# eriklindernoren/PyTorch-GAN

Measured on NVIDIA H100. Metric: DCGAN 64x64 images/sec (full G+D step), higher is better.
Workload: dtype tf32 (fp32 storage, fp32 accumulate)

## Files before the change

### include/b200gan.h

```cpp
#ifndef B200GAN_H
#define B200GAN_H

#include <stddef.h>
#include <stdint.h>

#ifdef __cplusplus
extern "C" {
#endif

#define B200GAN_VERSION 100

enum {
  B200GAN_OK = 0,
  B200GAN_E_UNSUPPORTED = -1,
  B200GAN_E_BAD_ARG = -2,
  B200GAN_E_CUDA = -3,
  B200GAN_E_ARCH = -4
};

enum { B200GAN_ACT_NONE = 0, B200GAN_ACT_LRELU = 1, B200GAN_ACT_RELU = 2, B200GAN_ACT_TANH = 3,
       B200GAN_ACT_SIGMOID = 4 };

enum { B200GAN_ALGO_AUTO = 0,
       B200GAN_ALGO_SIMT = 1,
// ... 32 lines not shown
  int32_t round_tf32;
} b200gan_epilogue;

int b200gan_version(void);
const char *b200gan_last_error(void);
int b200gan_check_device(void);

size_t b200gan_packed_weight_floats(const b200gan_conv_geom *g, int pack);
int b200gan_pack_weights(const b200gan_conv_geom *g, int pack, const float *w, float *packed,
                         void *stream);

typedef struct b200gan_pack_job {
  const float *w;
  float *packed;
  b200gan_conv_geom geom;
  int32_t pack;
} b200gan_pack_job;
int b200gan_pack_weights_multi(const b200gan_pack_job *jobs, int32_t count, void *stream);

int b200gan_conv2d_supported(const b200gan_conv_geom *g, int pass, int algo);

int b200gan_conv2d_fprop(const b200gan_conv_geom *g, const b200gan_epilogue *ep, const float *x,
                         const float *packed, float *y, int algo, void *stream);

size_t b200gan_conv2d_dgrad_workspace_floats(const b200gan_conv_geom *g, int algo);
int b200gan_conv2d_dgrad(const b200gan_conv_geom *g, const float *dy, const float *packed,
                         float *dx, float *workspace, int algo, void *stream);

size_t b200gan_conv2d_wgrad_workspace_floats(const b200gan_conv_geom *g, int algo);
int b200gan_conv2d_wgrad(const b200gan_conv_geom *g, const float *x, const float *dy, float *dw,
                         float *db, float *workspace, int algo, void *stream);
int b200gan_conv2d_wgrad_fused_bias(const b200gan_conv_geom *g, const float *x, const float *dy, float *dw,
                                    float *db, float *workspace, int algo, void *stream);

int b200gan_epilogue_bwd(const float *dy, const float *y, const float *chan_scale, int32_t act,
                         float slope, int64_t n, int32_t K, int64_t PQ, int32_t round_tf32,
                         float *dz, void *stream);

int b200gan_bias_grad(const float *dy, const float *y, const float *chan_scale, int32_t act, float slope,
                      int64_t rows, int32_t K, int64_t PQ, float *db, void *stream);

typedef struct b200gan_norm_desc {
  int32_t N, HW, C;
  int32_t per_sample;
  float eps;
  float momentum;
  int32_t act;
  float slope;
  int32_t round_tf32;
} b200gan_norm_desc;

int b200gan_norm_stats(const b200gan_norm_desc *d, const float *x, double *stats, void *stream);
int b200gan_norm_finalize(const b200gan_norm_desc *d, double *stats, const float *gamma,
                          const float *beta, float *mean_rstd, float *scale_shift,
                          float *running_mean, float *running_var, int64_t *num_batches_tracked,
                          void *stream);
int b200gan_norm_apply(const b200gan_norm_desc *d, const float *x, const float *scale_shift,
                       float *y, void *stream);
int b200gan_norm_bwd(const b200gan_norm_desc *d, const float *dy, const float *x, const float *y,
                     const float *mean_rstd, const float *scale_shift, const float *gamma, double *sums, float *dx,
                     float *dgamma_dbeta, void *stream);

int b200gan_norm_dbwd(const b200gan_norm_desc *d, const float *dy, const float *x, const float *mean_rstd,
                      const float *scale_shift, const float *gamma, const float *u, const float *ugamma_ubeta,
                      double *sums, float *gx, float *gdy, float *ggamma_per_group, void *stream);

// ... 172 lines not shown
```

### pytorch-gan_b200/b200gan/_lib.py

```python
import ctypes
import os

_HERE = os.path.dirname(os.path.abspath(__file__))
LIB_PATH = os.path.join(_HERE, "libb200gan.so")

c_i32, c_i64, c_f32, c_f64 = ctypes.c_int32, ctypes.c_int64, ctypes.c_float, ctypes.c_double
c_vp, c_sz = ctypes.c_void_p, ctypes.c_size_t

ACT_NONE, ACT_LRELU, ACT_RELU, ACT_TANH, ACT_SIGMOID = 0, 1, 2, 3, 4
ALGO_AUTO, ALGO_SIMT, ALGO_TC = 0, 1, 2
PAD_ZERO, PAD_REFLECT = 0, 1
PACK_SIMT_FPROP, PACK_SIMT_DGRAD, PACK_TC_FPROP, PACK_TC_DGRAD, PACK_TC_FPROP_UP2, PACK_TC_DGRAD_UP2 = range(6)


class ConvGeom(ctypes.Structure):
    _fields_ = [(n, c_i32) for n in (
        "N", "H", "W", "C", "K", "R", "S", "stride", "pad_t", "pad_l", "pad_b", "pad_r",
        "pad_mode", "up", "transposed", "P", "Q")]

    def key(self):
        return tuple(getattr(self, n) for n, _ in self._fields_)


class Epilogue(ctypes.Structure):
# ... 38 lines not shown
class TailDesc(ctypes.Structure):
    _fields_ = [("N", c_i32), ("H", c_i32), ("W", c_i32), ("C", c_i32), ("K", c_i32), ("act_mid", c_i32),
                ("slope", c_f32), ("act_out", c_i32)]


PIXEL_LOSS_MSE, PIXEL_LOSS_L1 = 0, 1
LAYOUT_NCHW, LAYOUT_NHWC = 0, 1


class PixelLossDesc(ctypes.Structure):
    _fields_ = [("mode", c_i32), ("layout_a", c_i32), ("layout_b", c_i32), ("reserved", c_i32), ("n", c_i64),
                ("N", c_i32), ("C", c_i32), ("H", c_i32), ("W", c_i32)]


class AdamTensor(ctypes.Structure):
    _fields_ = [("p", c_vp), ("g", c_vp), ("m", c_vp), ("v", c_vp), ("n", c_i64)]


_P = ctypes.POINTER
SIGNATURES = {
    "b200gan_version": (c_i32, []),
    "b200gan_last_error": (ctypes.c_char_p, []),
    "b200gan_check_device": (c_i32, []),
    "b200gan_packed_weight_floats": (c_sz, [_P(ConvGeom), c_i32]),
    "b200gan_pack_weights": (c_i32, [_P(ConvGeom), c_i32, c_vp, c_vp, c_vp]),
    "b200gan_pack_weights_multi": (c_i32, [_P(PackJob), c_i32, c_vp]),
    "b200gan_conv2d_supported": (c_i32, [_P(ConvGeom), c_i32, c_i32]),
    "b200gan_conv2d_fprop": (c_i32, [_P(ConvGeom), _P(Epilogue), c_vp, c_vp, c_vp, c_i32, c_vp]),
    "b200gan_conv2d_dgrad_workspace_floats": (c_sz, [_P(ConvGeom), c_i32]),
    "b200gan_conv2d_dgrad": (c_i32, [_P(ConvGeom), c_vp, c_vp, c_vp, c_vp, c_i32, c_vp]),
    "b200gan_conv2d_wgrad_workspace_floats": (c_sz, [_P(ConvGeom), c_i32]),
    "b200gan_conv2d_wgrad": (c_i32, [_P(ConvGeom), c_vp, c_vp, c_vp, c_vp, c_vp, c_i32, c_vp]),
    "b200gan_conv2d_wgrad_fused_bias": (c_i32, [_P(ConvGeom), c_vp, c_vp, c_vp, c_vp, c_vp, c_i32, c_vp]),
    "b200gan_epilogue_bwd": (c_i32, [c_vp, c_vp, c_vp, c_i32, c_f32, c_i64, c_i32, c_i64, c_i32, c_vp, c_vp]),
    "b200gan_bias_grad": (c_i32, [c_vp, c_vp, c_vp, c_i32, c_f32, c_i64, c_i32, c_i64, c_vp, c_vp]),
    "b200gan_norm_stats": (c_i32, [_P(NormDesc), c_vp, c_vp, c_vp]),
    "b200gan_norm_finalize": (c_i32, [_P(NormDesc), c_vp, c_vp, c_vp, c_vp, c_vp, c_vp, c_vp, c_vp, c_vp]),
    "b200gan_norm_apply": (c_i32, [_P(NormDesc), c_vp, c_vp, c_vp, c_vp]),
    "b200gan_norm_bwd": (c_i32, [_P(NormDesc), c_vp, c_vp, c_vp, c_vp, c_vp, c_vp, c_vp, c_vp, c_vp, c_vp]),
    "b200gan_norm_dbwd": (c_i32, [_P(NormDesc)] + [c_vp] * 12),
    "b200gan_conv2d_dgrad_norm_supported": (c_i32, [_P(ConvGeom)]),
    "b200gan_conv2d_dgrad_norm": (c_i32, [_P(ConvGeom), _P(NormDesc)] + [c_vp] * 8),
    "b200gan_norm_bwd_from_sums": (c_i32, [_P(NormDesc)] + [c_vp] * 9),
    "b200gan_tail_supported": (c_i32, [_P(TailDesc)]),
    "b200gan_tail_fprop": (c_i32, [_P(TailDesc), c_vp, c_vp, c_vp, c_vp, c_vp, c_vp]),
    "b200gan_tail_bwd_workspace_bytes": (c_sz, [_P(TailDesc)]),
    "b200gan_tail_bwd": (c_i32, [_P(TailDesc)] + [c_vp] * 10 + [c_i32, c_vp]),
    "b200gan_nchw_to_nhwc": (c_i32, [c_vp, c_vp, c_i32, c_i32, c_i32, c_vp]),
    "b200gan_nhwc_to_nchw": (c_i32, [c_vp, c_vp, c_i32, c_i32, c_i32, c_vp]),
    "b200gan_upsample2x_fwd": (c_i32, [c_vp, c_vp, c_i32, c_i32, c_i32, c_i32, c_vp]),
    "b200gan_upsample2x_bwd": (c_i32, [c_vp, c_vp, c_i32, c_i32, c_i32, c_i32, c_vp]),
    "b200gan_pad2d_fwd": (c_i32, [c_vp, c_vp] + [c_i32] * 10 + [c_vp]),
    "b200gan_pad2d_bwd": (c_i32, [c_vp, c_vp] + [c_i32] * 9 + [c_vp]),
    "b200gan_act_fwd": (c_i32, [c_vp, c_vp, c_i32, c_i32, c_f32, c_i64, c_i32, c_i64, c_vp, c_vp]),
    "b200gan_mlp_critic_fwd": (c_i32, [_P(MlpCriticDesc)] + [c_vp] * 13),
    "b200gan_mlp_critic_bwd_workspace_floats": (c_sz, [_P(MlpCriticDesc)]),
    "b200gan_mlp_critic_bwd": (c_i32, [_P(MlpCriticDesc)] + [c_vp] * 20),
    "b200gan_mlp_critic_dbwd_workspace_floats": (c_sz, [_P(MlpCriticDesc)]),
    "b200gan_mlp_critic_dbwd": (c_i32, [_P(MlpCriticDesc)] + [c_vp] * 15),
    "b200gan_critic_step_workspace_floats": (c_sz, [_P(MlpCriticDesc)]),
    "b200gan_critic_step_mlp": (c_i32, [_P(MlpCriticDesc), c_f32] + [c_vp] * 18),
    "b200gan_mlp_disc_fwd": (c_i32, [_P(MlpCriticDesc)] + [c_vp] * 13),
    "b200gan_mlp_disc_bwd_workspace_floats": (c_sz, [_P(MlpCriticDesc)]),
    "b200gan_mlp_disc_bwd": (c_i32, [_P(MlpCriticDesc)] + [c_vp] * 19),
    "b200gan_mlp_gen_saved_floats": (c_sz, [_P(MlpGenDesc)]),
    "b200gan_mlp_gen_workspace_floats": (c_sz, [_P(MlpGenDesc)]),
# ... 56 lines not shown
```

### pytorch-gan_b200/b200gan/ops.py

```python
import ctypes
import os

import torch

from . import _lib
from ._lib import (ACT_NONE, ALGO_AUTO, ALGO_SIMT, ALGO_TC, PACK_SIMT_DGRAD, PACK_SIMT_FPROP, PACK_TC_DGRAD,
                   PACK_TC_DGRAD_UP2, PACK_TC_FPROP, PACK_TC_FPROP_UP2, PAD_REFLECT, PAD_ZERO, ConvGeom, Epilogue,
                   MlpCriticDesc, MlpGenDesc, MlpGenGrads, NbBn, NormDesc, PixelLossDesc, TailDesc)

CL = torch.channels_last


class Config:
    algo = os.environ.get("B200GAN_ALGO", "auto")
    weight_cache = True
    contiguous_hw_limit = 64
    fuse_narrow_chain = os.environ.get("B200GAN_FUSE_CHAIN", "1") not in ("", "0")


def _stream():
    return torch.cuda.current_stream().cuda_stream


def _ptr(t):
# ... 106 lines not shown
def conv_fprop(g, x, packed, algo, bias=None, act=ACT_NONE, slope=0.0, chan_scale=None, stats=None,
               stats_per_sample=False, round_tf32=False):
    y = empty_cl(g.N, g.K, g.P, g.Q, x.device)
    if g.N == 0:
        return y
    ep = Epilogue()
    ep.bias, ep.act, ep.slope = _ptr(bias), act, slope
    ep.chan_scale, ep.stats = _ptr(chan_scale), _ptr(stats)
    ep.stats_per_sample, ep.round_tf32 = int(stats_per_sample), int(round_tf32)
    _lib.check(_lib.load().b200gan_conv2d_fprop(ctypes.byref(g), ctypes.byref(ep), x.data_ptr(), packed.data_ptr(),
                                                y.data_ptr(), algo, _stream()), "conv2d_fprop")
    return y


def conv_dgrad(g, dy, packed, algo):
    lib = _lib.load()
    dx = empty_cl(g.N, g.C, g.H, g.W, dy.device)
    nws = lib.b200gan_conv2d_dgrad_workspace_floats(ctypes.byref(g), algo)
    ws = torch.empty(nws, device=dy.device, dtype=torch.float32) if nws else None
    _lib.check(lib.b200gan_conv2d_dgrad(ctypes.byref(g), dy.data_ptr(), packed.data_ptr(), dx.data_ptr(), _ptr(ws),
                                        algo, _stream()), "conv2d_dgrad")
    return dx


def conv_wgrad(g, x, dy, weight_shape, need_bias, algo):
    lib = _lib.load()
    dw = torch.empty(weight_shape, device=x.device, dtype=torch.float32)
    db = torch.empty(g.K, device=x.device, dtype=torch.float32) if need_bias else None
    nws = lib.b200gan_conv2d_wgrad_workspace_floats(ctypes.byref(g), algo)
    ws = torch.empty(nws, device=x.device, dtype=torch.float32) if nws else None
    _lib.check(lib.b200gan_conv2d_wgrad_fused_bias(ctypes.byref(g), x.data_ptr(), dy.data_ptr(), dw.data_ptr(),
                                                   _ptr(db), _ptr(ws), algo, _stream()), "conv2d_wgrad")
    return dw, db


def epilogue_bwd(dy, y, chan_scale, act, slope, round_tf32=False):
    n, k, p, q = dy.shape
    dz = torch.empty_like(dy, memory_format=CL)
    _lib.check(_lib.load().b200gan_epilogue_bwd(dy.data_ptr(), _ptr(y), _ptr(chan_scale), act, slope, dy.numel(), k,
                                                p * q, int(round_tf32), dz.data_ptr(), _stream()), "epilogue_bwd")
    return dz


def bias_grad(dy, y, chan_scale, act, slope):
    n, k, p, q = dy.shape
    db = torch.empty(k, device=dy.device, dtype=torch.float32)
    _lib.check(_lib.load().b200gan_bias_grad(dy.data_ptr(), _ptr(y), _ptr(chan_scale), act, slope, n * p * q, k, p * q,
                                             db.data_ptr(), _stream()), "bias_grad")
    return db


def _norm_desc(shape, per_sample, eps, momentum, act, slope, round_tf32):
    n, c, h, w = shape
    d = NormDesc()
    d.N, d.HW, d.C, d.per_sample = n, h * w, c, int(per_sample)
    d.eps, d.momentum, d.act, d.slope, d.round_tf32 = eps, momentum, act, slope, int(round_tf32)
    return d


_zero_scratch = {}


def zero_scratch(device, numel):
    key = (device, numel)
    t = _zero_scratch.get(key)
    if t is None:
# ... 597 lines not shown
```

### pytorch-gan_b200/csrc/conv_api.cu

```cuda
#include "common.cuh"
#include <atomic>
#include <mutex>
#include <string.h>
#include <stdlib.h>

namespace b200gan {

int simt_gather_gemm(int N, int H, int W, int C, int P, int Q, int K, int R, int S, int stride,
                     int pad_t, int pad_l, int pad_mode, int up, int mode,
                     const b200gan_epilogue *ep, const float *x, const float *wp, float *y,
                     cudaStream_t st);
int simt_wgrad(int N, int H, int W, int Cg, int P, int Q, int Cd, int R, int S, int stride,
               int pad_t, int pad_l, int pad_mode, int up, const float *xg, const float *dn,
               float *dw, cudaStream_t st);
int simt_colsum(const float *x, float *out, int64_t M, int C, cudaStream_t st);
bool nb_wgrad_ok(const b200gan_conv_geom *g);
int nb_wgrad_run(const b200gan_conv_geom *g, const b200gan_nb_bn *in_bn, const float *x, const float *dz, float *dw,
                 float *workspace, cudaStream_t st);
size_t nb_wgrad_workspace_floats(const b200gan_conv_geom *g);
bool nb_plain_fprop_ok(const b200gan_conv_geom *g);
int nb_plain_fprop(const b200gan_conv_geom *g, const b200gan_epilogue *ep, const float *x, const float *packed, float *y,
                   cudaStream_t st);
bool nb_plain_dgrad_ok(const b200gan_conv_geom *g);
int nb_plain_dgrad(const b200gan_conv_geom *g, const float *dy, const float *packed, float *dx, cudaStream_t st);
bool fewk_ok(const b200gan_conv_geom *g, int pas);
int fewk_fprop(const b200gan_conv_geom *g, const b200gan_epilogue *ep, const float *x, const float *packed, float *y,
               cudaStream_t st);
int fewk_dgrad(const b200gan_conv_geom *g, const float *dy, const float *packed, float *dx, cudaStream_t st);
int fewk_wgrad(const b200gan_conv_geom *g, const float *x, const float *dy, float *dw, float *workspace, cudaStream_t st);
size_t fewk_wgrad_workspace_floats(const b200gan_conv_geom *g);
int tc_supported(const b200gan_conv_geom *g, int pass);
int tc_fprop(const b200gan_conv_geom *g, const b200gan_epilogue *ep, const float *x,
             const float *packed, float *y, cudaStream_t st);
struct TcNormBwd;
int tc_dgrad(const b200gan_conv_geom *g, const float *dy, const float *packed, float *dx, const TcNormBwd *nb,
             cudaStream_t st);
size_t tc_wgrad_workspace_floats(const b200gan_conv_geom *g);
int tc_wgrad(const b200gan_conv_geom *g, const float *x, const float *dy, float *dw, float *db, float *ws,
             cudaStream_t st);

static thread_local char g_err[512] = "";
void set_error(const char *fmt, ...) {
  va_list ap;
  va_start(ap, fmt);
  vsnprintf(g_err, sizeof(g_err), fmt, ap);
  va_end(ap);
}

int conv_stats_pass(const float *y, int N, int HW, int C, int per_sample, double *stats, cudaStream_t st) {
  b200gan_norm_desc nd;
  memset(&nd, 0, sizeof(nd));
  nd.N = N; nd.HW = HW; nd.C = C; nd.per_sample = per_sample;
  return b200gan_norm_stats(&nd, y, stats, st);
}

int num_sms() {
  static std::atomic<int> cache[64];
  int dev = 0;
  if (cudaGetDevice(&dev) != cudaSuccess || dev < 0 || dev >= 64) {
    cudaGetLastError();
    return 132;
  }
  int v = cache[dev].load(std::memory_order_relaxed);
  if (v > 0) return v;
  if (cudaDeviceGetAttribute(&v, cudaDevAttrMultiProcessorCount, dev) != cudaSuccess || v <= 0) {
    cudaGetLastError();
    return 132;
  }
  cache[dev].store(v, std::memory_order_relaxed);
  return v;
// ... 365 lines not shown

static int conv2d_wgrad(const b200gan_conv_geom *g, const float *x, const float *dy, float *dw, float *db,
                        float *workspace, int algo, bool fuse_db, void *stream) {
  if (int e = validate_geom(g)) return e;
  B2_CHECK_ARG(x && dy && dw, "conv2d_wgrad: null pointer");
  cudaStream_t st = as_stream(stream);
  int rc = B200GAN_OK;
  switch (wgrad_route(g, algo)) {
    case WgradRoute::Tc:
      if (!tc_supported(g, 2)) B2_UNSUPPORTED("conv2d_wgrad: geometry not supported by the tensor-core path");
      if (fuse_db && !g->transposed) return tc_wgrad(g, x, dy, dw, db, workspace, st);
      rc = tc_wgrad(g, x, dy, dw, nullptr, workspace, st);
      break;
    case WgradRoute::Fewk:
      rc = fewk_wgrad(g, x, dy, dw, workspace, st);
      break;
    case WgradRoute::Staged:
      rc = nb_wgrad_run(g, nullptr, x, dy, dw, workspace, st);
      break;
    case WgradRoute::Simt:
      if (g->transposed)
        rc = simt_wgrad(g->N, g->P, g->Q, g->K, g->H, g->W, g->C, g->R, g->S, g->stride, g->pad_t, g->pad_l,
                        B200GAN_PAD_ZERO, 1, dy, x, dw, st);
      else
        rc = simt_wgrad(g->N, g->H, g->W, g->C, g->P, g->Q, g->K, g->R, g->S, g->stride, g->pad_t, g->pad_l,
                        g->pad_mode, g->up, x, dy, dw, st);
      break;
  }
  if (rc) return rc;
  if (db) return simt_colsum(dy, db, (int64_t)g->N * g->P * g->Q, g->K, st);
  return B200GAN_OK;
}

extern "C" int b200gan_conv2d_wgrad(const b200gan_conv_geom *g, const float *x, const float *dy, float *dw,
                                    float *db, float *workspace, int algo, void *stream) {
  return conv2d_wgrad(g, x, dy, dw, db, workspace, algo, false, stream);
}

extern "C" int b200gan_conv2d_wgrad_fused_bias(const b200gan_conv_geom *g, const float *x, const float *dy, float *dw,
                                               float *db, float *workspace, int algo, void *stream) {
  return conv2d_wgrad(g, x, dy, dw, db, workspace, algo, true, stream);
}
```

### pytorch-gan_b200/csrc/wgrad_tc.cu

```cuda
#include "tc_common.cuh"
#include <stdlib.h>

namespace b200gan {

constexpr int WG_THREADS = 384;
constexpr int WG_MAX_JOBS = 52;
constexpr int WG_PIX = 32;
constexpr int WG_CHUNK_BYTES = WG_PIX * 128;

struct WgJob {
  int16_t s_dc, d_dc;
  int8_t s_da, d_da;
  int8_t s_dw, s_dh;
  int8_t db;
  int8_t pad_;
};

struct WgParams {
  WgJob jobs[WG_MAX_JOBS];
  int32_t njobs;
  int32_t bw_log2, bh_log2;
  int32_t tiles_w, tiles_h, N;
  int32_t imgs_per_box;
  int32_t tiles_total, tiles_per_split;
  int32_t s_is_a;
  int32_t mtiles, ntiles;
  int32_t ldn;
  int32_t mtotal;
  float *partial;
  float *db;
};

template <int NB, int STAGES>
struct WgSmem {
  static constexpr int A_BYTES = 4 * WG_CHUNK_BYTES;
  static constexpr int B_BYTES = (NB / 32) * WG_CHUNK_BYTES;
  static constexpr int STAGE_BYTES = A_BYTES + B_BYTES;
  static constexpr int RING = STAGES * STAGE_BYTES;
  static constexpr int T_BYTES = NB * 128;
  static constexpr int STAGING = (NB / 32) * 16384;
  static constexpr int MAIN = RING + 2 * T_BYTES > STAGING ? RING + 2 * T_BYTES : STAGING;
  static constexpr int TOTAL = MAIN + 1024 + 256;
  static_assert(TOTAL <= 232448, "wgrad_tc_kernel: shared memory");
};

__device__ __forceinline__ void wg_consumers_sync() { asm volatile("bar.sync 1, 256;" ::: "memory"); }

__device__ __forceinline__ int wg_kpos(int p) { return (p & ~7) | ((p & 7) >> 1) | ((p & 1) << 2); }

template <int NB, int STAGES>
__global__ void __launch_bounds__(WG_THREADS, 1)
wgrad_tc_kernel(const __grid_constant__ CUtensorMap tmX, const __grid_constant__ CUtensorMap tmY,
                const __grid_constant__ CUtensorMap tmP, const __grid_constant__ WgParams p) {
  using L = WgSmem<NB, STAGES>;
  extern __shared__ uint8_t smem_raw[];
  uint8_t *smem = reinterpret_cast<uint8_t *>((reinterpret_cast<uintptr_t>(smem_raw) + 1023) & ~(uintptr_t)1023);
  uint64_t *full = reinterpret_cast<uint64_t *>(smem + L::MAIN);
  uint64_t *empty = full + STAGES;

  const int warp = threadIdx.x >> 5, lane = threadIdx.x & 31;
  const int split = blockIdx.x, job = blockIdx.y;
  const int mt = blockIdx.z / p.ntiles, nt = blockIdx.z % p.ntiles;
  const int t_begin = split * p.tiles_per_split;
  int t_end = t_begin + p.tiles_per_split;
  if (t_end > p.tiles_total) t_end = p.tiles_total;
  const int iters = t_end - t_begin;

  if (threadIdx.x == 0) {
    tma_prefetch_desc(&tmX);
    tma_prefetch_desc(&tmY);
    for (int s = 0; s < STAGES; ++s) {
      mbar_init(&full[s], 1);
      mbar_init(&empty[s], 256);
    }
    fence_barrier_init();
  }
  __syncthreads();

  if (warp < 4) {
    setmaxnreg_dec<40>();
    if (warp == 0 && lane == 0) {
      const WgJob jb = p.jobs[job];
      const CUtensorMap *mapA = p.s_is_a ? &tmX : &tmY;
      const CUtensorMap *mapB = p.s_is_a ? &tmY : &tmX;
      const int a_dc = p.s_is_a ? jb.s_dc : jb.d_dc, a_da = p.s_is_a ? jb.s_da : jb.d_da;
      const int a_dw = p.s_is_a ? jb.s_dw : 0, a_dh = p.s_is_a ? jb.s_dh : 0;
      const int b_dc = p.s_is_a ? jb.d_dc : jb.s_dc, b_da = p.s_is_a ? jb.d_da : jb.s_da;
      const int b_dw = p.s_is_a ? 0 : jb.s_dw, b_dh = p.s_is_a ? 0 : jb.s_dh;
      int stage = 0;
      uint32_t phase = 0;
      for (int it = 0; it < iters; ++it) {
        int t = t_begin + it;
        const int tw = t % p.tiles_w;
        t /= p.tiles_w;
        const int th = t % p.tiles_h;
        const int n = (t / p.tiles_h) * p.imgs_per_box;
        const int w0 = tw << p.bw_log2, h0 = th << p.bh_log2;
        mbar_wait(&empty[stage], phase ^ 1);
        uint8_t *sa = smem + stage * L::STAGE_BYTES;
        uint8_t *sb = sa + L::A_BYTES;
        mbar_arrive_expect_tx(&full[stage], L::STAGE_BYTES);
#pragma unroll
        for (int c = 0; c < 4; ++c)
          tma_load_5d(sa + c * WG_CHUNK_BYTES, mapA, &full[stage], a_dc + (mt * 4 + c) * 32, w0 + a_dw, a_da,
                      h0 + a_dh, n);
#pragma unroll
        for (int c = 0; c < NB / 32; ++c)
          tma_load_5d(sb + c * WG_CHUNK_BYTES, mapB, &full[stage], b_dc + (nt * (NB / 32) + c) * 32, w0 + b_dw, b_da,
                      h0 + b_dh, n);
        if (++stage == STAGES) {
          stage = 0;
          phase ^= 1;
        }
      }
    }
  } else {
    setmaxnreg_inc<232>();
    if (iters == 0) return;
    const int ct = threadIdx.x - 128;
    const int half = ct >> 7;
    const int tp = ct & 31, tq = ct >> 5;
    const int tk = wg_kpos(tp);
    const int wq = tq & 3;
    const int ac = 16 * (wq & 1) + (lane >> 2), ap = 2 * (lane & 3);
    const int abase = (2 * half + (wq >> 1)) * WG_CHUNK_BYTES + ap * 128 + (ac & 3) * 4;
    const uint32_t aoff[4] = {
        (uint32_t)(abase + ((((ac >> 2)) ^ ap) << 4)),
        (uint32_t)(abase + ((((ac >> 2) + 2) ^ ap) << 4)),
        (uint32_t)(abase + 128 + ((((ac >> 2)) ^ (ap + 1)) << 4)),
        (uint32_t)(abase + 128 + ((((ac >> 2) + 2) ^ (ap + 1)) << 4))};
    float acc[NB / 2];
    const bool db_job = p.db != nullptr && p.jobs[job].db;
    const bool dbA = db_job && !p.s_is_a && nt == 0;
    const bool dbB = db_job && p.s_is_a && mt == 0;
    float dsa0 = 0.f, dsa1 = 0.f;
    float dsb[NB <= 64 ? NB / 8 : 1];
#pragma unroll
    for (int i = 0; i < (NB <= 64 ? NB / 8 : 1); ++i) dsb[i] = 0.f;
    int stage = 0;
    uint32_t phase = 0;
    auto prepare = [&](int it, uint32_t(&fa)[16]) {
      uint8_t *tb = smem + L::RING + (it & 1) * L::T_BYTES;
      mbar_wait(&full[stage], phase);
      wg_consumers_sync();
      const uint8_t *src = smem + stage * L::STAGE_BYTES;
#pragma unroll
      for (int k = 0; k < WG_PIX / 8; ++k)
#pragma unroll
        for (int j = 0; j < 4; ++j) fa[4 * k + j] = *reinterpret_cast<const uint32_t *>(src + aoff[j] + k * 1024);
      if (dbA) {
#pragma unroll
        for (int k = 0; k < WG_PIX / 8; ++k) {
          dsa0 += __uint_as_float(fa[4 * k]) + __uint_as_float(fa[4 * k + 2]);
          dsa1 += __uint_as_float(fa[4 * k + 1]) + __uint_as_float(fa[4 * k + 3]);
        }
      }
#pragma unroll
      for (int c = 0; c < NB / 32; ++c) {
        const float4 v = *reinterpret_cast<const float4 *>(src + L::A_BYTES + c * WG_CHUNK_BYTES + tp * 128 +
                                                           ((tq ^ (tp & 7)) << 4));
        const float e[4] = {v.x, v.y, v.z, v.w};
        if constexpr (NB <= 64) {
          if (dbB) {
#pragma unroll
            for (int i = 0; i < 4; ++i) dsb[4 * c + i] += e[i];
          }
        }
#pragma unroll
        for (int i = 0; i < 4; ++i) {
          const int r = c * 32 + tq * 4 + i;
          *reinterpret_cast<float *>(tb + r * 128 + (((tk >> 2) ^ (r & 7)) << 4) + (tk & 3) * 4) = e[i];
        }
      }
      mbar_arrive(&empty[stage]);
      fence_proxy_async();
      wg_consumers_sync();
      if (++stage == STAGES) {
        stage = 0;
        phase ^= 1;
      }
    };
    auto mma = [&](int it, const uint32_t(&fa)[16]) {
      const uint32_t sb = smem_u32(smem + L::RING + (it & 1) * L::T_BYTES);
      wgmma_fence();
#pragma unroll
      for (int k = 0; k < WG_PIX / 8; ++k)
        wgmma_tf32_rs<NB>(acc, fa + 4 * k, gmma_desc_sw128(sb + k * 32), (it > 0 || k > 0) ? 1u : 0u);
      wgmma_commit();
    };
    uint32_t fa0[16], fa1[16];
    prepare(0, fa0);
#pragma unroll 1
    for (int it = 0; it < iters; it += 2) {
      mma(it, fa0);
      if (it + 1 < iters) prepare(it + 1, fa1);
      wgmma_wait<0>();
      if (it + 1 < iters) {
        mma(it + 1, fa1);
        if (it + 2 < iters) prepare(it + 2, fa0);
        wgmma_wait<0>();
      }
    }
    wgmma_wait<0>();
    wgmma_fence_regs<NB / 2>(acc);
    if (dbA) {
      dsa0 += __shfl_xor_sync(0xffffffffu, dsa0, 1);
      dsa1 += __shfl_xor_sync(0xffffffffu, dsa1, 1);
      dsa0 += __shfl_xor_sync(0xffffffffu, dsa0, 2);
      dsa1 += __shfl_xor_sync(0xffffffffu, dsa1, 2);
      if ((lane & 3) == 0) {
        const int ch = (mt * 4 + 2 * half + (wq >> 1)) * 32 + ac;
        atomicAdd(p.db + ch, dsa0);
        atomicAdd(p.db + ch + 8, dsa1);
      }
    }
    if constexpr (NB <= 64) {
      if (dbB) {
#pragma unroll
        for (int i = 0; i < NB / 8; ++i) {
          float s = dsb[i];
#pragma unroll
          for (int o = 16; o > 0; o >>= 1) s += __shfl_xor_sync(0xffffffffu, s, o);
          if (lane == 0) atomicAdd(p.db + nt * NB + (i >> 2) * 32 + tq * 4 + (i & 3), s);
        }
      }
    }
    wg_consumers_sync();
    store_acc_sw128<NB>(smem, acc, half * 64);
    fence_proxy_async();
    wg_consumers_sync();
    if (ct == 0) {
      const int row0 = job * p.mtotal + mt * 128;
#pragma unroll 1
      for (int c = 0; c < NB; c += 32) tma_reduce_add_2d(&tmP, smem + (c >> 5) * 16384, nt * NB + c, row0);
      tma_store_commit_and_wait_read();
    }
  }
}

struct WgReduceP {
  int32_t K, C, R, S, njobs, s_is_a, up2, transposed;
  int32_t mtotal, ldn;
};
__device__ __forceinline__ bool up2_contrib(int r, int a, int d) {
  if (a == 0) return d == 0 ? r == 0 : r >= 1;
  return d == 0 ? r <= 1 : r == 2;
}
__global__ void wgrad_reduce_kernel(const float *__restrict__ partial, float *__restrict__ dw, WgReduceP p) {
  int64_t total = (int64_t)p.K * p.C * p.R * p.S;
  for (int64_t i = (int64_t)blockIdx.x * blockDim.x + threadIdx.x; i < total;
       i += (int64_t)gridDim.x * blockDim.x) {
    int c = (int)(i % p.C);
    int64_t t = i / p.C;
    int k = (int)(t % p.K);
    t /= p.K;
    int s = (int)(t % p.S), r = (int)(t / p.S);
    const int sch = p.transposed ? k : c;
    const int dch = p.transposed ? c : k;
    int64_t elem = p.s_is_a ? (int64_t)sch * p.ldn + dch : (int64_t)dch * p.ldn + sch;
// ... 40 lines not shown
    const int t = e % RS;
    int cl, rw;
    if (col_is_b) { cl = (e / RS) % WR_COL; rw = e / (RS * WR_COL); }
    else          { rw = (e / RS) % WR_ROW; cl = e / (RS * WR_ROW); }
    const int col = col0 + cl, row = row0 + rw;
    if (col >= ncol || row >= nrow) continue;
    float acc;
    if (!p.up2) {
      acc = s[rw][cl][t];
    } else {
      const int r = t / 3, q = t % 3;
      acc = 0.f;
#pragma unroll
      for (int j = 0; j < 16; ++j) {
        const int ph = j >> 2, tp = j & 3;
        if (up2_contrib(r, ph >> 1, tp >> 1) && up2_contrib(q, ph & 1, tp & 1)) acc += s[rw][cl][j];
      }
    }
    const int a = col_is_b ? row : col, b = col_is_b ? col : row;
    dw[((int64_t)a * nb + b) * RS + t] = acc;
  }
}

static int ilog2c(int v) {
  int l = 0;
  while ((1 << l) < v) ++l;
  return l;
}

struct WgPlan {
  int s_is_a, NB, mtiles, ntiles, mtotal, ldn, njobs, bwl, bhl, tiles_w, tiles_h, tiles_total, nsplits, tps, Ho, Wo;
  int sch, dch;
  int ipb;
};

static bool wg_plan(const b200gan_conv_geom *g, WgPlan &pl) {
  if (g->pad_mode != B200GAN_PAD_ZERO || g->N < 1) return false;
  if (g->stride != 1 && g->stride != 2) return false;
  if (g->C % 32 || g->K % 32 || 2 * g->C > 32767 || 2 * g->K > 32767) return false;
  const bool up2 = g->up == 2;
  if (up2 && (g->transposed || g->stride != 1 ||
              !(g->R == 3 && g->S == 3 && g->pad_t == 1 && g->pad_l == 1 && g->pad_b == 1 && g->pad_r == 1)))
    return false;
  if (g->R * g->S > WG_MAX_JOBS || g->R > 15 || g->S > 15 || g->pad_t > 15 || g->pad_l > 15) return false;
  pl.sch = g->transposed ? g->K : g->C;
  pl.dch = g->transposed ? g->C : g->K;
  if (g->stride == 2) {
    const int Hf = g->transposed ? g->P : g->H, Wf = g->transposed ? g->Q : g->W;
    if ((Hf & 1) || (Wf & 1)) return false;
  }
  if (pl.dch % 128 == 0) pl.s_is_a = 0;
  else if (pl.sch % 128 == 0) pl.s_is_a = 1;
  else return false;
  const int mch = pl.s_is_a ? pl.sch : pl.dch, nch = pl.s_is_a ? pl.dch : pl.sch;
  pl.NB = nch % 128 == 0 ? 128 : (nch % 64 == 0 ? 64 : 32);
  if (nch % 256 == 0) pl.NB = 256;
  pl.mtotal = mch;
  pl.ldn = nch;
  pl.mtiles = mch / 128;
  pl.ntiles = nch / pl.NB;
  pl.njobs = up2 ? 16 : g->R * g->S;
  pl.Ho = up2 ? g->H : (g->transposed ? g->H : g->P);
  pl.Wo = up2 ? g->W : (g->transposed ? g->W : g->Q);
  const int pl2 = 5;
  pl.bwl = ilog2c(pl.Wo);
  if (pl.bwl > pl2) pl.bwl = pl2;
  pl.bhl = ilog2c(pl.Ho);
  if (pl.bhl > pl2 - pl.bwl) pl.bhl = pl2 - pl.bwl;
  pl.tiles_w = ceil_div(pl.Wo, 1 << pl.bwl);
  pl.tiles_h = ceil_div(pl.Ho, 1 << pl.bhl);
  pl.ipb = WG_PIX >> (pl.bwl + pl.bhl);
  int64_t tt = (int64_t)ceil_div(g->N, pl.ipb) * pl.tiles_w * pl.tiles_h;
  if (tt > (1 << 30)) return false;
  pl.tiles_total = (int)tt;
  const int64_t ctas_per_split = (int64_t)pl.njobs * pl.mtiles * pl.ntiles;
  int max_ns = pl.tiles_total / 8;
  if (max_ns < 1) max_ns = 1;
  if (max_ns > 4 * num_sms()) max_ns = 4 * num_sms();
  int ns = 1;
  int64_t best = -1;
  for (int s = 1; s <= max_ns; ++s) {
    const int64_t waves = ceil_div64(s * ctas_per_split, num_sms());
    const int64_t cost = waves * (ceil_div(pl.tiles_total, s) + 8);
    if (best < 0 || cost < best) {
      best = cost;
      ns = s;
    }
  }
  pl.tps = ceil_div(pl.tiles_total, ns);
  pl.nsplits = ceil_div(pl.tiles_total, pl.tps);
  return true;
}

int tc_wgrad_supported(const b200gan_conv_geom *g) {
  WgPlan pl;
  return wg_plan(g, pl) ? 1 : 0;
}

size_t tc_wgrad_workspace_floats(const b200gan_conv_geom *g) {
  WgPlan pl;
  if (!wg_plan(g, pl)) return 0;
  return (size_t)pl.njobs * pl.mtotal * pl.ldn;
}

template <int NB, int STAGES>
static int launch_wg(const CUtensorMap &tmX, const CUtensorMap &tmY, const CUtensorMap &tmP, const WgParams &p, dim3 grid,
                     cudaStream_t st) {
  constexpr int SMEM = WgSmem<NB, STAGES>::TOTAL;
  static std::atomic<uint64_t> attr_done{0};
  if (int e = ensure_dynamic_smem(wgrad_tc_kernel<NB, STAGES>, SMEM, attr_done)) return e;
  wgrad_tc_kernel<NB, STAGES><<<grid, WG_THREADS, SMEM, st>>>(tmX, tmY, tmP, p);
  B2_LAUNCH_CHECK();
  return B200GAN_OK;
}

int tc_wgrad(const b200gan_conv_geom *g, const float *x, const float *dy, float *dw, float *db, float *ws,
             cudaStream_t st) {
  WgPlan pl;
  if (!wg_plan(g, pl)) B2_UNSUPPORTED("tensor-core wgrad: geometry not supported");
  B2_CHECK_ARG(ws != nullptr, "tensor-core wgrad: workspace required");
  B2_CHECK_ARG(!(db && g->transposed), "tensor-core wgrad: bias gradient of a ConvTranspose2d is not fused");
  B2_CHECK_ARG(((uintptr_t)x % 16 == 0) && ((uintptr_t)dy % 16 == 0) && ((uintptr_t)ws % 16 == 0),
               "tensor-core wgrad: pointers must be 16-byte aligned");
  const bool up2 = g->up == 2;
  const int st2 = g->stride == 2;
  WgParams p;
  memset(&p, 0, sizeof(p));
  p.njobs = pl.njobs;
  if (up2) {
    for (int ph = 0; ph < 4; ++ph)
      for (int tp = 0; tp < 4; ++tp) {
        int a = ph >> 1, b = ph & 1, dr = tp >> 1, ds = tp & 1;
        WgJob &j = p.jobs[ph * 4 + tp];
        j.d_dc = (int16_t)(b * g->K); j.d_da = (int8_t)a; j.s_dh = (int8_t)(a - 1 + dr); j.s_dw = (int8_t)(b - 1 + ds);
        j.db = tp == 0;
      }
  } else {
    p.jobs[0].db = 1;
    for (int r = 0; r < g->R; ++r)
      for (int s2 = 0; s2 < g->S; ++s2) {
        WgJob &j = p.jobs[r * g->S + s2];
        const int eh = r - g->pad_t, ew = s2 - g->pad_l;
        if (!st2) {
          j.s_dh = (int8_t)eh; j.s_dw = (int8_t)ew;
        } else {
          j.s_dh = (int8_t)(eh >= 0 ? eh / 2 : -((-eh + 1) / 2)); j.s_da = (int8_t)(eh & 1);
          j.s_dw = (int8_t)(ew >= 0 ? ew / 2 : -((-ew + 1) / 2)); j.s_dc = (int16_t)((ew & 1) * pl.sch);
        }
      }
  }
  p.bw_log2 = pl.bwl; p.bh_log2 = pl.bhl;
  p.tiles_w = pl.tiles_w; p.tiles_h = pl.tiles_h; p.N = g->N; p.imgs_per_box = pl.ipb;
  p.tiles_total = pl.tiles_total; p.tiles_per_split = pl.tps;
  p.s_is_a = pl.s_is_a; p.mtiles = pl.mtiles; p.ntiles = pl.ntiles; p.ldn = pl.ldn; p.mtotal = pl.mtotal;
  p.partial = ws;
  p.db = db;

  const float *sptr = g->transposed ? dy : x, *dptr = g->transposed ? x : dy;
  const uint64_t Hs = g->transposed ? g->P : g->H, Ws = g->transposed ? g->Q : g->W, Cs = pl.sch;
  const uint64_t Hd = g->transposed ? g->H : g->P, Wd = g->transposed ? g->W : g->Q, Cd = pl.dch;
  CUtensorMap tmX, tmY;
  const uint32_t box[5] = {32, (uint32_t)(1 << pl.bwl), 1, (uint32_t)(1 << pl.bhl), (uint32_t)pl.ipb};
  {
    uint64_t dims[5], strides[4];
    if (!st2) {
      dims[0] = Cs; dims[1] = Ws; dims[2] = 1; dims[3] = Hs; dims[4] = g->N;
      strides[0] = Cs * 4; strides[1] = Ws * Cs * 4; strides[2] = Ws * Cs * 4; strides[3] = Hs * Ws * Cs * 4;
    } else {
      dims[0] = 2 * Cs; dims[1] = Ws / 2; dims[2] = 2; dims[3] = Hs / 2; dims[4] = g->N;
      strides[0] = 2 * Cs * 4; strides[1] = Ws * Cs * 4; strides[2] = 2 * Ws * Cs * 4; strides[3] = Hs * Ws * Cs * 4;
    }
    if (int e = make_tmap_f32(&tmX, sptr, 5, dims, strides, box)) return e;
  }
  {
    uint64_t dims[5], strides[4];
    if (!up2) {
      dims[0] = Cd; dims[1] = Wd; dims[2] = 1; dims[3] = Hd; dims[4] = g->N;
      strides[0] = Cd * 4; strides[1] = Wd * Cd * 4; strides[2] = Wd * Cd * 4; strides[3] = Hd * Wd * Cd * 4;
    } else {
      dims[0] = 2 * Cd; dims[1] = Wd / 2; dims[2] = 2; dims[3] = Hd / 2; dims[4] = g->N;
      strides[0] = 2 * Cd * 4; strides[1] = Wd * Cd * 4; strides[2] = 2 * Wd * Cd * 4; strides[3] = Hd * Wd * Cd * 4;
    }
    if (int e = make_tmap_f32(&tmY, dptr, 5, dims, strides, box)) return e;
  }
  CUtensorMap tmP;
  {
    uint64_t dims[2] = {(uint64_t)pl.ldn, (uint64_t)pl.njobs * pl.mtotal};
    uint64_t strides[1] = {(uint64_t)pl.ldn * 4};
    uint32_t pbox[2] = {32, 128};
    if (int e = make_tmap_f32(&tmP, ws, 2, dims, strides, pbox)) return e;
  }
  B2_CUDA(cudaMemsetAsync(ws, 0, (size_t)pl.njobs * pl.mtotal * pl.ldn * sizeof(float), st));
  if (db) B2_CUDA(cudaMemsetAsync(db, 0, (size_t)g->K * sizeof(float), st));
  dim3 grid((unsigned)pl.nsplits, (unsigned)pl.njobs, (unsigned)(pl.mtiles * pl.ntiles));
  int rc = pl.NB == 256 ? launch_wg<256, 3>(tmX, tmY, tmP, p, grid, st)
           : pl.NB == 128 ? launch_wg<128, 6>(tmX, tmY, tmP, p, grid, st)
           : pl.NB == 64 ? launch_wg<64, 8>(tmX, tmY, tmP, p, grid, st)
                         : launch_wg<32, 8>(tmX, tmY, tmP, p, grid, st);
  if (rc) return rc;
  WgReduceP rp;
  rp.K = g->K; rp.C = g->C; rp.R = g->R; rp.S = g->S; rp.njobs = pl.njobs;
  rp.s_is_a = pl.s_is_a; rp.up2 = up2 ? 1 : 0; rp.transposed = g->transposed ? 1 : 0; rp.mtotal = pl.mtotal; rp.ldn = pl.ldn;
  int64_t total = (int64_t)g->K * g->C * g->R * g->S;
  if (g->R * g->S <= WR_TAPS && g->K >= 32 && g->C >= 32) {
    const bool col_is_k = (pl.s_is_a != 0) != (g->transposed != 0);
// ... 14 lines not shown
```

Measured before the change: 48610.

## Add phase-major wgrad path that loads one halo tile and reuses it across four taps

For the upsample-by-2 weight-gradient case where the source is the A operand, each CTA now handles four kernel taps (one phase group) at once. It loads a single haloed A tile (box enlarged by one in width and height) and the B tile once, then issues four register-sourced wgmma accumulations from shifted shared-memory offsets, instead of one job per tap each reloading its own tiles. The intent is to cut redundant TMA traffic and B transposes by a factor of four per tap group. In exchange it uses four accumulator sets (more register pressure), splits the tile range into quarters across blockIdx.y, and adds a separate ring layout with fewer stages.

Measured after the change: 50460, median of 6. +3.8%, better.

```diff
diff --git a/include/b200gan.h b/include/b200gan.h
--- a/include/b200gan.h
+++ b/include/b200gan.h
@@ -88,6 +88,7 @@
                          float *db, float *workspace, int algo, void *stream);
 int b200gan_conv2d_wgrad_fused_bias(const b200gan_conv_geom *g, const float *x, const float *dy, float *dw,
                                     float *db, float *workspace, int algo, void *stream);
+int b200gan_conv2d_wgrad_phase_major(const b200gan_conv_geom *g);
 
 int b200gan_epilogue_bwd(const float *dy, const float *y, const float *chan_scale, int32_t act,
                          float slope, int64_t n, int32_t K, int64_t PQ, int32_t round_tf32,
diff --git a/pytorch-gan_b200/b200gan/_lib.py b/pytorch-gan_b200/b200gan/_lib.py
--- a/pytorch-gan_b200/b200gan/_lib.py
+++ b/pytorch-gan_b200/b200gan/_lib.py
@@ -94,6 +94,7 @@
     "b200gan_conv2d_wgrad_workspace_floats": (c_sz, [_P(ConvGeom), c_i32]),
     "b200gan_conv2d_wgrad": (c_i32, [_P(ConvGeom), c_vp, c_vp, c_vp, c_vp, c_vp, c_i32, c_vp]),
     "b200gan_conv2d_wgrad_fused_bias": (c_i32, [_P(ConvGeom), c_vp, c_vp, c_vp, c_vp, c_vp, c_i32, c_vp]),
+    "b200gan_conv2d_wgrad_phase_major": (c_i32, [_P(ConvGeom)]),
     "b200gan_epilogue_bwd": (c_i32, [c_vp, c_vp, c_vp, c_i32, c_f32, c_i64, c_i32, c_i64, c_i32, c_vp, c_vp]),
     "b200gan_bias_grad": (c_i32, [c_vp, c_vp, c_vp, c_i32, c_f32, c_i64, c_i32, c_i64, c_vp, c_vp]),
     "b200gan_norm_stats": (c_i32, [_P(NormDesc), c_vp, c_vp, c_vp]),
diff --git a/pytorch-gan_b200/b200gan/ops.py b/pytorch-gan_b200/b200gan/ops.py
--- a/pytorch-gan_b200/b200gan/ops.py
+++ b/pytorch-gan_b200/b200gan/ops.py
@@ -162,6 +162,10 @@
     _lib.check(lib.b200gan_conv2d_wgrad_fused_bias(ctypes.byref(g), x.data_ptr(), dy.data_ptr(), dw.data_ptr(),
                                                    _ptr(db), _ptr(ws), algo, _stream()), "conv2d_wgrad")
     return dw, db
+
+
+def conv_wgrad_phase_major(g):
+    return bool(_lib.load().b200gan_conv2d_wgrad_phase_major(ctypes.byref(g)))
 
 
 def epilogue_bwd(dy, y, chan_scale, act, slope, round_tf32=False):
diff --git a/pytorch-gan_b200/csrc/conv_api.cu b/pytorch-gan_b200/csrc/conv_api.cu
--- a/pytorch-gan_b200/csrc/conv_api.cu
+++ b/pytorch-gan_b200/csrc/conv_api.cu
@@ -36,6 +36,7 @@
 int tc_dgrad(const b200gan_conv_geom *g, const float *dy, const float *packed, float *dx, const TcNormBwd *nb,
              cudaStream_t st);
 size_t tc_wgrad_workspace_floats(const b200gan_conv_geom *g);
+int tc_wgrad_phase_major(const b200gan_conv_geom *g);
 int tc_wgrad(const b200gan_conv_geom *g, const float *x, const float *dy, float *dw, float *db, float *ws,
              cudaStream_t st);
 
@@ -467,6 +468,11 @@
   return B200GAN_OK;
 }
 
+extern "C" int b200gan_conv2d_wgrad_phase_major(const b200gan_conv_geom *g) {
+  if (!g || validate_geom(g) || !tc_supported(g, 2)) return 0;
+  return tc_wgrad_phase_major(g);
+}
+
 extern "C" int b200gan_conv2d_wgrad(const b200gan_conv_geom *g, const float *x, const float *dy, float *dw,
                                     float *db, float *workspace, int algo, void *stream) {
   return conv2d_wgrad(g, x, dy, dw, db, workspace, algo, false, stream);
diff --git a/pytorch-gan_b200/csrc/wgrad_tc.cu b/pytorch-gan_b200/csrc/wgrad_tc.cu
--- a/pytorch-gan_b200/csrc/wgrad_tc.cu
+++ b/pytorch-gan_b200/csrc/wgrad_tc.cu
@@ -7,6 +7,8 @@
 constexpr int WG_MAX_JOBS = 52;
 constexpr int WG_PIX = 32;
 constexpr int WG_CHUNK_BYTES = WG_PIX * 128;
+constexpr int WG_PH_STAGES = 4;
+constexpr int WG_HALO_BYTES = 9216;
 
 struct WgJob {
   int16_t s_dc, d_dc;
@@ -24,6 +26,7 @@
   int32_t imgs_per_box;
   int32_t tiles_total, tiles_per_split;
   int32_t s_is_a;
+  int32_t phase_major;
   int32_t mtiles, ntiles;
   int32_t ldn;
   int32_t mtotal;
@@ -42,11 +45,42 @@
   static constexpr int MAIN = RING + 2 * T_BYTES > STAGING ? RING + 2 * T_BYTES : STAGING;
   static constexpr int TOTAL = MAIN + 1024 + 256;
   static_assert(TOTAL <= 232448, "wgrad_tc_kernel: shared memory");
+  static constexpr int PH_A_BYTES = 4 * WG_HALO_BYTES;
+  static constexpr int PH_STAGE_BYTES = PH_A_BYTES + B_BYTES;
+  static_assert(NB > 64 || (WG_PH_STAGES * PH_STAGE_BYTES <= RING && 4 * STAGING <= RING),
+                "wgrad_tc_kernel: phase-major ring");
 };
 
+__device__ __forceinline__ uint32_t wg_lds32(uint32_t addr) {
+  uint32_t v;
+  asm volatile("ld.shared.b32 %0, [%1];" : "=r"(v) : "r"(addr));
+  return v;
+}
+
 __device__ __forceinline__ void wg_consumers_sync() { asm volatile("bar.sync 1, 256;" ::: "memory"); }
 
 __device__ __forceinline__ int wg_kpos(int p) { return (p & ~7) | ((p & 7) >> 1) | ((p & 1) << 2); }
+
+template <int NB>
+__device__ __forceinline__ void wg_transpose_b(const uint8_t *src, uint8_t *tb, int tp, int tq, int tk, bool db,
+                                               float *dsb) {
+#pragma unroll
+  for (int c = 0; c < NB / 32; ++c) {
+    const float4 v = *reinterpret_cast<const float4 *>(src + c * WG_CHUNK_BYTES + tp * 128 + ((tq ^ (tp & 7)) << 4));
+    const float e[4] = {v.x, v.y, v.z, v.w};
+    if constexpr (NB <= 64) {
+      if (db) {
+#pragma unroll
+        for (int i = 0; i < 4; ++i) dsb[4 * c + i] += e[i];
+      }
+    }
+#pragma unroll
+    for (int i = 0; i < 4; ++i) {
+      const int r = c * 32 + tq * 4 + i;
+      *reinterpret_cast<float *>(tb + r * 128 + (((tk >> 2) ^ (r & 7)) << 4) + (tk & 3) * 4) = e[i];
+    }
+  }
+}
 
 template <int NB, int STAGES>
 __global__ void __launch_bounds__(WG_THREADS, 1)
@@ -59,12 +93,19 @@
   uint64_t *empty = full + STAGES;
 
   const int warp = threadIdx.x >> 5, lane = threadIdx.x & 31;
-  const int split = blockIdx.x, job = blockIdx.y;
+  const bool phm = NB <= 64 && p.phase_major;
+  const int split = blockIdx.x;
+  const int job = phm ? blockIdx.y & ~3 : blockIdx.y;
   const int mt = blockIdx.z / p.ntiles, nt = blockIdx.z % p.ntiles;
-  const int t_begin = split * p.tiles_per_split;
+  int t_begin = split * p.tiles_per_split;
   int t_end = t_begin + p.tiles_per_split;
   if (t_end > p.tiles_total) t_end = p.tiles_total;
-  const int iters = t_end - t_begin;
+  if (phm) {
+    const int qn = (t_end - t_begin + 3) >> 2;
+    t_begin += (blockIdx.y & 3) * qn;
+    if (t_end > t_begin + qn) t_end = t_begin + qn;
+  }
+  const int iters = t_end > t_begin ? t_end - t_begin : 0;
 
   if (threadIdx.x == 0) {
     tma_prefetch_desc(&tmX);
@@ -87,6 +128,11 @@
       const int a_dw = p.s_is_a ? jb.s_dw : 0, a_dh = p.s_is_a ? jb.s_dh : 0;
       const int b_dc = p.s_is_a ? jb.d_dc : jb.s_dc, b_da = p.s_is_a ? jb.d_da : jb.s_da;
       const int b_dw = p.s_is_a ? 0 : jb.s_dw, b_dh = p.s_is_a ? 0 : jb.s_dh;
+      const int nst = phm ? WG_PH_STAGES : STAGES;
+      const int a_pitch = phm ? WG_HALO_BYTES : WG_CHUNK_BYTES;
+      const int stage_bytes = phm ? L::PH_STAGE_BYTES : L::STAGE_BYTES;
+      const uint32_t tx = phm ? 4 * 128 * ((1 << p.bw_log2) + 1) * ((1 << p.bh_log2) + 1) * p.imgs_per_box + L::B_BYTES
+                              : L::STAGE_BYTES;
       int stage = 0;
       uint32_t phase = 0;
       for (int it = 0; it < iters; ++it) {
@@ -97,18 +143,18 @@
         const int n = (t / p.tiles_h) * p.imgs_per_box;
         const int w0 = tw << p.bw_log2, h0 = th << p.bh_log2;
         mbar_wait(&empty[stage], phase ^ 1);
-        uint8_t *sa = smem + stage * L::STAGE_BYTES;
-        uint8_t *sb = sa + L::A_BYTES;
-        mbar_arrive_expect_tx(&full[stage], L::STAGE_BYTES);
+        uint8_t *sa = smem + stage * stage_bytes;
+        uint8_t *sb = sa + 4 * a_pitch;
+        mbar_arrive_expect_tx(&full[stage], tx);
 #pragma unroll
         for (int c = 0; c < 4; ++c)
-          tma_load_5d(sa + c * WG_CHUNK_BYTES, mapA, &full[stage], a_dc + (mt * 4 + c) * 32, w0 + a_dw, a_da,
+          tma_load_5d(sa + c * a_pitch, mapA, &full[stage], a_dc + (mt * 4 + c) * 32, w0 + a_dw, a_da,
                       h0 + a_dh, n);
 #pragma unroll
         for (int c = 0; c < NB / 32; ++c)
           tma_load_5d(sb + c * WG_CHUNK_BYTES, mapB, &full[stage], b_dc + (nt * (NB / 32) + c) * 32, w0 + b_dw, b_da,
                       h0 + b_dh, n);
-        if (++stage == STAGES) {
+        if (++stage == nst) {
           stage = 0;
           phase ^= 1;
         }
@@ -137,8 +183,101 @@
     float dsb[NB <= 64 ? NB / 8 : 1];
 #pragma unroll
     for (int i = 0; i < (NB <= 64 ? NB / 8 : 1); ++i) dsb[i] = 0.f;
+    auto flush_dsb = [&]() {
+      if constexpr (NB <= 64) {
+        if (dbB) {
+#pragma unroll
+          for (int i = 0; i < NB / 8; ++i) {
+            float s = dsb[i];
+#pragma unroll
+            for (int o = 16; o > 0; o >>= 1) s += __shfl_xor_sync(0xffffffffu, s, o);
+            if (lane == 0) atomicAdd(p.db + nt * NB + (i >> 2) * 32 + tq * 4 + (i & 3), s);
+          }
+        }
+      }
+    };
     int stage = 0;
     uint32_t phase = 0;
+    if constexpr (NB <= 64) {
+      if (phm) {
+        uint32_t hoff[WG_PIX / 8][4];
+#pragma unroll
+        for (int k = 0; k < WG_PIX / 8; ++k) {
+          const int q = 8 * k, r = q >> p.bw_log2, img = r >> p.bh_log2;
+          const int row0 = q + r + img * ((1 << p.bw_log2) + 1) + ap;
+#pragma unroll
+          for (int j = 0; j < 4; ++j) {
+            const int row = row0 + j;
+            hoff[k][j] = (uint32_t)((2 * half + (wq >> 1)) * WG_HALO_BYTES + row * 128 + (((ac >> 2) ^ (row & 7)) << 4) +
+                                    (ac & 3) * 4);
+          }
+        }
+        const int bw_bytes = 128 << p.bw_log2;
+        float acc4[4][NB / 2];
+        uint32_t fa[2][16];
+        auto transpose = [&](int it) {
+          mbar_wait(&full[stage], phase);
+          wg_consumers_sync();
+          wg_transpose_b<NB>(smem + stage * L::PH_STAGE_BYTES + L::PH_A_BYTES, smem + L::RING + (it & 1) * L::T_BYTES,
+                             tp, tq, tk, dbB, dsb);
+          fence_proxy_async();
+          wg_consumers_sync();
+        };
+        auto taps = [&](int it) {
+          const uint32_t xs = smem_u32(smem) + stage * L::PH_STAGE_BYTES;
+          const uint32_t sb = smem_u32(smem + L::RING + (it & 1) * L::T_BYTES);
+#pragma unroll
+          for (int t = 0; t < 4; ++t) {
+            const int j0 = (t >> 1) + (t & 1);
+            const uint32_t xt = xs + (t >> 1) * bw_bytes;
+            uint32_t *f = fa[t & 1];
+            wgmma_wait<1>();
+#pragma unroll
+            for (int k = 0; k < WG_PIX / 8; ++k) {
+              f[4 * k + 0] = wg_lds32(xt + hoff[k][j0]);
+              f[4 * k + 1] = wg_lds32(xt + (hoff[k][j0] ^ 32));
+              f[4 * k + 2] = wg_lds32(xt + hoff[k][j0 + 1]);
+              f[4 * k + 3] = wg_lds32(xt + (hoff[k][j0 + 1] ^ 32));
+            }
+            wgmma_fence();
+#pragma unroll
+            for (int k = 0; k < WG_PIX / 8; ++k)
+              wgmma_tf32_rs<NB>(acc4[t], f + 4 * k, gmma_desc_sw128(sb + k * 32), (it > 0 || k > 0) ? 1u : 0u);
+            wgmma_commit();
+          }
+          mbar_arrive(&empty[stage]);
+          if (++stage == WG_PH_STAGES) {
+            stage = 0;
+            phase ^= 1;
+          }
+        };
+        transpose(0);
+#pragma unroll 1
+        for (int it = 0; it < iters; ++it) {
+          taps(it);
+          if (it + 1 < iters) transpose(it + 1);
+        }
+        wgmma_wait<0>();
+#pragma unroll
+        for (int t = 0; t < 4; ++t) wgmma_fence_regs<NB / 2>(acc4[t]);
+        flush_dsb();
+        wg_consumers_sync();
+#pragma unroll
+        for (int t = 0; t < 4; ++t) store_acc_sw128<NB>(smem + t * L::STAGING, acc4[t], half * 64);
+        fence_proxy_async();
+        wg_consumers_sync();
+        if (ct == 0) {
+#pragma unroll 1
+          for (int t = 0; t < 4; ++t) {
+            const int row0 = (job + t) * p.mtotal + mt * 128;
+            for (int c = 0; c < NB; c += 32)
+              tma_reduce_add_2d(&tmP, smem + t * L::STAGING + (c >> 5) * 16384, nt * NB + c, row0);
+          }
+          tma_store_commit_and_wait_read();
+        }
+        return;
+      }
+    }
     auto prepare = [&](int it, uint32_t(&fa)[16]) {
       uint8_t *tb = smem + L::RING + (it & 1) * L::T_BYTES;
       mbar_wait(&full[stage], phase);
@@ -155,23 +294,7 @@
           dsa1 += __uint_as_float(fa[4 * k + 1]) + __uint_as_float(fa[4 * k + 3]);
         }
       }
-#pragma unroll
-      for (int c = 0; c < NB / 32; ++c) {
-        const float4 v = *reinterpret_cast<const float4 *>(src + L::A_BYTES + c * WG_CHUNK_BYTES + tp * 128 +
-                                                           ((tq ^ (tp & 7)) << 4));
-        const float e[4] = {v.x, v.y, v.z, v.w};
-        if constexpr (NB <= 64) {
-          if (dbB) {
-#pragma unroll
-            for (int i = 0; i < 4; ++i) dsb[4 * c + i] += e[i];
-          }
-        }
-#pragma unroll
-        for (int i = 0; i < 4; ++i) {
-          const int r = c * 32 + tq * 4 + i;
-          *reinterpret_cast<float *>(tb + r * 128 + (((tk >> 2) ^ (r & 7)) << 4) + (tk & 3) * 4) = e[i];
-        }
-      }
+      wg_transpose_b<NB>(src + L::A_BYTES, tb, tp, tq, tk, dbB, dsb);
       mbar_arrive(&empty[stage]);
       fence_proxy_async();
       wg_consumers_sync();
@@ -214,17 +337,7 @@
         atomicAdd(p.db + ch + 8, dsa1);
       }
     }
-    if constexpr (NB <= 64) {
-      if (dbB) {
-#pragma unroll
-        for (int i = 0; i < NB / 8; ++i) {
-          float s = dsb[i];
-#pragma unroll
-          for (int o = 16; o > 0; o >>= 1) s += __shfl_xor_sync(0xffffffffu, s, o);
-          if (lane == 0) atomicAdd(p.db + nt * NB + (i >> 2) * 32 + tq * 4 + (i & 3), s);
-        }
-      }
-    }
+    flush_dsb();
     wg_consumers_sync();
     store_acc_sw128<NB>(smem, acc, half * 64);
     fence_proxy_async();
@@ -331,6 +444,7 @@
   int s_is_a, NB, mtiles, ntiles, mtotal, ldn, njobs, bwl, bhl, tiles_w, tiles_h, tiles_total, nsplits, tps, Ho, Wo;
   int sch, dch;
   int ipb;
+  int phase_major;
 };
 
 static bool wg_plan(const b200gan_conv_geom *g, WgPlan &pl) {
@@ -388,12 +502,18 @@
   }
   pl.tps = ceil_div(pl.tiles_total, ns);
   pl.nsplits = ceil_div(pl.tiles_total, pl.tps);
+  pl.phase_major = up2 && pl.s_is_a && pl.bwl >= 3;
   return true;
 }
 
 int tc_wgrad_supported(const b200gan_conv_geom *g) {
   WgPlan pl;
   return wg_plan(g, pl) ? 1 : 0;
+}
+
+int tc_wgrad_phase_major(const b200gan_conv_geom *g) {
+  WgPlan pl;
+  return wg_plan(g, pl) && pl.phase_major ? 1 : 0;
 }
 
 size_t tc_wgrad_workspace_floats(const b200gan_conv_geom *g) {
@@ -451,7 +571,7 @@
   p.bw_log2 = pl.bwl; p.bh_log2 = pl.bhl;
   p.tiles_w = pl.tiles_w; p.tiles_h = pl.tiles_h; p.N = g->N; p.imgs_per_box = pl.ipb;
   p.tiles_total = pl.tiles_total; p.tiles_per_split = pl.tps;
-  p.s_is_a = pl.s_is_a; p.mtiles = pl.mtiles; p.ntiles = pl.ntiles; p.ldn = pl.ldn; p.mtotal = pl.mtotal;
+  p.s_is_a = pl.s_is_a; p.phase_major = pl.phase_major; p.mtiles = pl.mtiles; p.ntiles = pl.ntiles; p.ldn = pl.ldn; p.mtotal = pl.mtotal;
   p.partial = ws;
   p.db = db;
 
@@ -469,7 +589,8 @@
       dims[0] = 2 * Cs; dims[1] = Ws / 2; dims[2] = 2; dims[3] = Hs / 2; dims[4] = g->N;
       strides[0] = 2 * Cs * 4; strides[1] = Ws * Cs * 4; strides[2] = 2 * Ws * Cs * 4; strides[3] = Hs * Ws * Cs * 4;
     }
-    if (int e = make_tmap_f32(&tmX, sptr, 5, dims, strides, box)) return e;
+    const uint32_t hbox[5] = {32, (uint32_t)(1 << pl.bwl) + 1, 1, (uint32_t)(1 << pl.bhl) + 1, (uint32_t)pl.ipb};
+    if (int e = make_tmap_f32(&tmX, sptr, 5, dims, strides, pl.phase_major ? hbox : box)) return e;
   }
   {
     uint64_t dims[5], strides[4];
```
